# GANtastic3/MaskCycleGAN-VC

Hardware: AMD Instinct MI355X
Metric: train iters/s (full G+D step), 80x64 mel bs=1 (higher is better)
Workload: dtype f32

## Files before the change

include/mcvc.h:

```cpp
#ifndef MCVC_H
#define MCVC_H

#ifdef __cplusplus
extern "C" {
#endif

#define MCVC_ABI_VERSION 3
#define MCVC_GEN_NPARAMS 110
#define MCVC_DISC_NPARAMS 20
#define MCVC_N_MEL 80

int mcvc_version(void);

int mcvc_set_deterministic(int on);
int mcvc_get_deterministic(void);
int mcvc_set_precise(int on);
int mcvc_get_precise(void);
int mcvc_set_trunk_persistent(int on);

int mcvc_twin_begin(void);
int mcvc_twin_switch(void);
int mcvc_twin_end(void);
int mcvc_twin_launches(void);

// ... 125 lines not shown
                     long long scratch_floats, int N, int H, int W, int Cin, int Cout, int branches, int KH, int KW, int stride,
                     int pad_h, int pad_w, int scheme, void* stream);
int mcvc_layer_wgrad(const float* x, const float* dy, float* dw0, float* dw1, float* scratch, long long scratch_floats, int N, int H,
                     int W, int Cin, int Cout, int branches, int KH, int KW, int stride, int pad_h, int pad_w, int scheme, void* stream);
int mcvc_trunk_layer_backward(const float* dy, const float* conv_out, const float* stats, const float* gamma, const float* beta,
                              const float* gamma_gate, const float* beta_gate, const float* w, const float* w_gate, const float* x_in,
                              float* dx, float* dconv, float* dgamma, float* dbeta, float* dgamma_gate, float* dbeta_gate, float* dw,
                              float* dw_gate, float* wpack, int B, int Cin, int T4, int Cout, int KW, void* stream);

int mcvc_instnorm_act_forward(float* x, const float* gamma, const float* beta, const float* gamma_gate,
                              const float* beta_gate, const float* residual, float* y, float* stats,
                              int N, int C, int H, int W, int act, void* stream);
int mcvc_instnorm_act_backward(const float* x, const float* gamma, const float* beta, const float* gamma_gate,
                               const float* beta_gate, const float* stats, float* dy, float* dx,
                               float* dgamma, float* dbeta, float* dgamma_gate, float* dbeta_gate,
                               int N, int C, int H, int W, int act, void* stream);

int mcvc_trunk_layer_forward(const float* x, const float* w, const float* bias, const float* gamma, const float* beta, const float* w_gate,
                             const float* bias_gate, const float* gamma_gate, const float* beta_gate, const float* residual, float* conv_out,
                             float* stats, float* y, int B, int Cin, int T4, int Cout, int KW, void* stream);

int mcvc_batched_gemm(const float* a, const float* b, float* c, int nbatch, int M, int N, int K, int lda, int ldb, int ldc,
                      long long a_stride, long long b_stride, long long c_stride, void* stream);

int mcvc_bias_grad(const float* dy, float* db, int N, int C, int P, void* stream);
int mcvc_act_forward(float* x, float* y, int N, int C, int P, int act, void* stream);
int mcvc_act_backward(const float* x, float* dy, float* dx, int N, int C, int P, int act, void* stream);
int mcvc_fif_input(const float* x, const float* mask, float* xin, int N, int P, void* stream);
int mcvc_fif_input_grad(const float* dxin, const float* mask, float* dx, int N, int P, int accumulate, void* stream);

int mcvc_trace_enable(int on);
int mcvc_trace_kinds(void);
const char* mcvc_trace_kind_name(int kind);
int mcvc_trace_collect(double* out);
int mcvc_trace_collect_raw(double* out, int max_records);

#ifdef __cplusplus
}
#endif
#endif
```

maskcyclegan-vc_amd/csrc/net.hip:

```cpp
#include "mcvc_common.h"
#include "twin.h"
#include "pack.h"
#include "misc.h"
#include "trunk.h"
#include "wino.h"
#include "wino4.h"
#include "sgemm.h"
#include "sampler.h"
#include "audio.h"
#include "../../include/mcvc.h"
#include <string.h>
#include <algorithm>
#include <map>
#include <mutex>
#include <vector>

static int g_deterministic = [] { const char* e = getenv("MCVC_DETERMINISTIC"); return (e && atoi(e) != 0) ? 1 : 0; }();
int mcvc_deterministic() { return g_deterministic; }

namespace {

constexpr float kInEps = 1e-5f;

struct View { float* p; long long sb, sc; int sh; };
// ... 2802 lines not shown
    if (!x || !w || !bias || !gamma || !beta || !conv_out || !stats || !y) return MCVC_ERR_INVALID;
    const int mode = w_gate ? TRUNK_IN_GLU : TRUNK_IN;
    if (!mcvc_trunk_applies(Cin, KW, Cout, B, T4, mode, 1)) return MCVC_ERR_INVALID;
    TrunkArgs a{};
    a.a0 = w; a.bias0 = bias; a.gamma0 = gamma; a.beta0 = beta;
    a.a1 = w_gate; a.bias1 = bias_gate; a.gamma1 = gamma_gate; a.beta1 = beta_gate;
    a.x = x; a.x_sc = (long long)B * T4; a.x_sb = T4;
    a.Cin = Cin; a.KW = KW; a.K = Cin * KW; a.M = Cout; a.Mtot = w_gate ? 2 * Cout : Cout; a.B = B; a.T4 = T4; a.N = B * T4;
    a.conv_out = conv_out; a.c_sc = (long long)B * T4; a.c_sb = T4;
    a.stats = stats; a.y = y; a.res = residual; a.y_sn = T4; a.y_sc = (long long)B * T4; a.eps = kInEps; a.mode = mode;
    return mcvc_trunk_launch(a, 1, (hipStream_t)stream);
}

int mcvc_batched_gemm(const float* a, const float* b, float* c, int nbatch, int M, int N, int K, int lda, int ldb, int ldc,
                      long long a_stride, long long b_stride, long long c_stride, void* stream)
{
    if (!a || !b || !c || nbatch < 1) return MCVC_ERR_INVALID;
    WinoGemmArgs ga{};
    ga.a = a; ga.a_xi = a_stride; ga.lda = lda; ga.b = b; ga.b_xi = b_stride; ga.ldb = ldb; ga.c = c; ga.c_xi = c_stride; ga.ldc = ldc;
    ga.M = M; ga.N = N; ga.K = K; ga.nxi = nbatch;
    return mcvc_wino_gemm_launch(ga, (hipStream_t)stream);
}

int mcvc_bias_grad(const float* dy, float* db, int N, int C, int P, void* stream)
{
    return mcvc_bias_grad_launch(dy, (long long)C * P, (long long)P, N, C, P, db, (hipStream_t)stream);
}

int mcvc_act_forward(float* x, float* y, int N, int C, int P, int act, void* stream)
{
    Exec ex{}; ex.s = (hipStream_t)stream;
    act_fwd(ex, x, 0, 1, y, N, C, P, act);
    return ex.err;
}

int mcvc_act_backward(const float* x, float* dy, float* dx, int N, int C, int P, int act, void* stream)
{
    Exec ex{}; ex.s = (hipStream_t)stream;
    act_bwd(ex, x, dy, 0, 1, dx, N, C, P, act);
    return ex.err;
}

int mcvc_fif_input(const float* x, const float* mask, float* xin, int N, int P, void* stream)
{
    return mcvc_prep_input_launch(x, mask, xin, N, P, (hipStream_t)stream);
}
// ... 8 lines not shown
```

maskcyclegan-vc_amd/csrc/wino.h:

```cpp
#pragma once
#include <hip/hip_runtime.h>

struct WinoXformArgs {
    const float* x; long long x_sb, x_sc; int x_sh;
    float* v;
    int N, C, H, W;
    int TH, TW, NT;
    int NTp;
    int pad;
};

struct WinoOutArgs {
    const float* m;
    const float* bias;
    float* y; long long y_sb, y_sc; int y_sh;
    int N, Cout, OH, OW, TH, TW, NT, NTp;
    int shuffle, YH, YW;
    int accumulate;
};

int mcvc_wino_input_launch(const WinoXformArgs& a, hipStream_t s);
struct NormArgs;
bool mcvc_norm_fwd_wino_applies(const NormArgs& a, const WinoOutArgs& w, int pts);
int mcvc_norm_fwd_wino_launch(const NormArgs& a, const WinoOutArgs& w, int pts, hipStream_t s);
// ... 39 lines not shown
        grow(colv, o);
#pragma unroll
        for (int aa = 0; aa < 6; ++aa) d0[(long long)(aa * 6 + b) * xi_stride] = o[aa];
    }
}
static __device__ __forceinline__ void wino_weight_tile(const float* w, float* dst, int Cout, int Cin, int ld, long long xi_stride, int co_off, int dgrad, int bx, int by)
{
    const int a_idx = bx * 256 + threadIdx.x;
    const int b_idx = by;
    const int co = dgrad ? b_idx : a_idx, ci = dgrad ? a_idx : b_idx;
    if (co >= Cout || ci >= Cin) return;
    wino_weight_core(w + ((long long)co * Cin + ci) * 25, dst, co, ci, ld, xi_stride, co_off, dgrad);
}


struct WinoGemmArgs {
    const float* a; long long a_xi; int lda;
    const float* b; long long b_xi; int ldb;
    float* c; long long c_xi; int ldc;
    int M, N, K;
    int nxi;
    int nt, mt;
    int mgroup;
};
int mcvc_wino_gemm_launch(const WinoGemmArgs& a, hipStream_t s);

template <int P>
static __device__ __forceinline__ void wino_g3(float v0, float v1, float v2, float* o)
{
    if constexpr (P == 4) { o[0] = v0; o[1] = 0.5f * (v0 + v1 + v2); o[2] = 0.5f * (v0 - v1 + v2); o[3] = v2; }
    else {
        const float e = v0 + v2, e2 = v0 * (1.0f / 24.0f) + v2 * (1.0f / 6.0f);
        o[0] = 0.25f * v0; o[1] = -(e + v1) * (1.0f / 6.0f); o[2] = -(e - v1) * (1.0f / 6.0f);
        o[3] = e2 + v1 * (1.0f / 12.0f); o[4] = e2 - v1 * (1.0f / 12.0f); o[5] = v2;
    }
}

template <int P>
static __device__ __forceinline__ void wino3_weight_core_p(const float* g, float* dst, int co, int ci, int ld, long long xi_stride, int co_off)
{
    float gg[5][5];
#pragma unroll
    for (int k = 0; k < 25; ++k) gg[k / 5][k % 5] = g[k];
#pragma unroll
    for (int qh = 0; qh < 2; ++qh)
#pragma unroll
        for (int qw = 0; qw < 2; ++qw) {
            float t[3][P];
// ... 78 lines not shown
```

maskcyclegan-vc_amd/csrc/wino_kernels.hip:

```cpp
#include "mcvc_common.h"
#include "trace.h"
#include "launch.h"
#include "wino.h"

namespace {

__device__ __forceinline__ void bt6(const float d[6], float o[6])
{
    o[0] = 4.f * d[0] - 5.f * d[2] + d[4];
    o[1] = -4.f * (d[1] + d[2]) + d[3] + d[4];
    o[2] = 4.f * (d[1] - d[2]) - d[3] + d[4];
    o[3] = -2.f * d[1] - d[2] + 2.f * d[3] + d[4];
    o[4] = 2.f * d[1] - d[2] - 2.f * d[3] + d[4];
    o[5] = 4.f * d[1] - 5.f * d[3] + d[5];
}

__global__ void __launch_bounds__(256) wino_input_kernel(const Twin<WinoXformArgs> tw)
{
    const WinoXformArgs a = tw.v[blockIdx.z];
    const int tile = blockIdx.x * 256 + threadIdx.x;
    const int c = blockIdx.y;
    if (tile >= a.NT) return;
    const int per = a.TH * a.TW;
    const int n = tile / per, r = tile - n * per;
// ... 434 lines not shown
        float o0, o1;
        at6(u[i], o0, o1);
        const float ov[2] = {o0 + bias, o1 + bias};
        const int oh = 2 * ty + i;
#pragma unroll
        for (int j = 0; j < 2; ++j) {
            const int ow = 2 * tx + j;
            if (oh >= a.OH || ow >= a.OW) continue;
            long long off;
            if (a.shuffle) {
                const int yh = 2 * oh + ((co >> 1) & 1), yw = 2 * ow + (co & 1);
                if (yh >= a.YH || yw >= a.YW) continue;
                off = (long long)(co >> 2) * a.y_sc + (long long)yh * a.y_sh + yw;
            } else {
                off = (long long)co * a.y_sc + (long long)oh * a.y_sh + ow;
            }
            if (a.accumulate) yn[off] += ov[j]; else yn[off] = ov[j];
        }
    }
}


constexpr int kGK = 16;
constexpr int kGStages = 4;
#ifndef MCVC_FOLDK
#define MCVC_FOLDK 32
#endif
constexpr int kFoldK = MCVC_FOLDK;
constexpr int kGA = kGK * 128;

__device__ __forceinline__ void wg_glds16(const float* g, float* l)
{
    __builtin_amdgcn_global_load_lds((const __attribute__((address_space(1))) void*)g,
                                     (__attribute__((address_space(3))) void*)l, 16, 0, 0);
}

template <int BN>
__global__ void __launch_bounds__(256, (BN == 64 ? 3 : 4)) wino_gemm_kernel(const Twin<WinoGemmArgs> tw)
{
    const WinoGemmArgs a = tw.v[blockIdx.z];
    constexpr int kGB = kGK * BN;
    constexpr int kGStage = kGA + kGB;
    constexpr int NACC = (BN == 64) ? 2 : 1;
    extern __shared__ __attribute__((aligned(16))) float smem[];
    const int tid = threadIdx.x, lane = tid & 63;
    const int wave = __builtin_amdgcn_readfirstlane(tid >> 6);
    const int l31 = lane & 31, half = lane >> 5;
    const int wm = (BN == 64) ? (wave >> 1) : wave, wn = (BN == 64) ? (wave & 1) : 0;
    int lid;
    {
        const int total = (int)gridDim.x, linear = (int)blockIdx.x;
        const int q = total >> 3, r = total & 7, xcd = linear & 7, k = linear >> 3;
        lid = (xcd < r ? xcd * (q + 1) : r * (q + 1) + (xcd - r) * q) + k;
    }
    const int n0 = (lid % a.nt) * BN; lid /= a.nt;
    const int m0 = (lid % a.mt) * 128;
    const int xi = lid / a.mt;
    const float* A = a.a + (long long)xi * a.a_xi + m0;
    const float* B = a.b + (long long)xi * a.b_xi + n0;
    const int fa0 = wave * 64 + lane, fa1 = fa0 + 256;
    const float* a_src0 = A + (long long)(fa0 >> 5) * a.lda + 4 * (fa0 & 31);
    const float* a_src1 = A + (long long)(fa1 >> 5) * a.lda + 4 * (fa1 & 31);
    const int bw = (BN == 64) ? wave : (wave & 1);
    const int fb = bw * 64 + lane;
    constexpr int F4R = BN / 4;
    int bcol = 4 * (fb % F4R);
    if (n0 + bcol > a.ldb - 4) bcol = a.ldb - 4 - n0;
    const float* b_src = B + (long long)(fb / F4R) * a.ldb + bcol;
    const long long a_step = (long long)kGK * a.lda, b_step = (long long)kGK * a.ldb;
    auto issue = [&](int stage_k, int buf) {
        float* base = smem + buf * kGStage;
        wg_glds16(a_src0 + stage_k * a_step, base + (wave * 64) * 4);
        wg_glds16(a_src1 + stage_k * a_step, base + (wave * 64 + 256) * 4);
        wg_glds16(b_src + stage_k * b_step, base + kGA + (bw * 64) * 4);
    };
    f32x16 acc[NACC], tot[NACC];
#pragma unroll
    for (int i = 0; i < NACC; ++i)
#pragma unroll
        for (int r = 0; r < 16; ++r) { acc[i][r] = 0.f; tot[i][r] = 0.f; }
    constexpr int kFoldSt = kFoldK / kGK;
    const int nst = a.K / kGK;
#pragma unroll
    for (int s = 0; s < kGStages - 1; ++s)
        if (s < nst) issue(s, s);
    const int a_lane = half * 128 + wm * (32 * NACC) + l31;
    const int b_lane = kGA + half * BN + wn * 32 + l31;
    for (int st = 0; st < nst; ++st) {
        const int newer = (nst - 1 - st) < (kGStages - 2) ? (nst - 1 - st) : (kGStages - 2);
        if (newer >= 2) __builtin_amdgcn_s_waitcnt(0x0F76);
        else if (newer == 1) __builtin_amdgcn_s_waitcnt(0x0F73);
        else __builtin_amdgcn_s_waitcnt(0x0F70);
        __builtin_amdgcn_s_barrier();
        if (st + kGStages - 1 < nst) issue(st + kGStages - 1, (st + kGStages - 1) % kGStages);
        if (st != 0 && (st % kFoldSt) == 0) {
#pragma unroll
            for (int i = 0; i < NACC; ++i)
#pragma unroll
                for (int r = 0; r < 16; ++r) { tot[i][r] += acc[i][r]; acc[i][r] = 0.f; }
        }
        const float* sb = smem + (st % kGStages) * kGStage;
        if constexpr (BN == 64) {
            float a0 = sb[a_lane], a1 = sb[a_lane + 32], b0 = sb[b_lane];
#pragma unroll
            for (int p = 0; p < kGK / 2; ++p) {
                const int q = (p + 1 < kGK / 2) ? p + 1 : p;
                const float na0 = sb[a_lane + q * 256], na1 = sb[a_lane + q * 256 + 32], nb0 = sb[b_lane + q * 2 * BN];
                acc[0] = __builtin_amdgcn_mfma_f32_32x32x2f32(a0, b0, acc[0], 0, 0, 0);
                acc[1] = __builtin_amdgcn_mfma_f32_32x32x2f32(a1, b0, acc[1], 0, 0, 0);
                __builtin_amdgcn_sched_group_barrier(0x100, 3, 0);
                __builtin_amdgcn_sched_group_barrier(0x008, 2, 0);
                a0 = na0; a1 = na1; b0 = nb0;
            }
        } else {
            float a0 = sb[a_lane], b0 = sb[b_lane];
#pragma unroll
            for (int p = 0; p < kGK / 2; ++p) {
                const int q = (p + 1 < kGK / 2) ? p + 1 : p;
                const float na0 = sb[a_lane + q * 256], nb0 = sb[b_lane + q * 2 * BN];
                acc[0] = __builtin_amdgcn_mfma_f32_32x32x2f32(a0, b0, acc[0], 0, 0, 0);
                __builtin_amdgcn_sched_group_barrier(0x100, 2, 0);
                __builtin_amdgcn_sched_group_barrier(0x008, 1, 0);
                a0 = na0; b0 = nb0;
            }
        }
    }
    const int n = n0 + wn * 32 + l31;
    const long long ldc = a.ldc;
    if (n < a.N) {
        float* C = a.c + (long long)xi * a.c_xi + n + (long long)(m0 + wm * (32 * NACC) + 4 * half) * ldc;
#pragma unroll
        for (int i = 0; i < NACC; ++i)
#pragma unroll
            for (int r = 0; r < 16; ++r) C[(long long)(i * 32 + (r & 3) + 8 * (r >> 2)) * ldc] = tot[i][r] + acc[i][r];
    }
}

template <int N> __device__ __forceinline__ void wait_vm() { __builtin_amdgcn_s_waitcnt(0x0F70 | (N & 15) | ((N >> 4) << 14)); }

template <int BM, int BN, int GK, int ST>
__global__ void __launch_bounds__(256) gemm2_kernel(const Twin<WinoGemmArgs> tw)
{
    const WinoGemmArgs a = tw.v[blockIdx.z];
    constexpr int SA = GK * BM, SB = GK * BN, STAGE = SA + SB;
    constexpr bool W22 = (BN % 64) == 0;
    constexpr int NBM = W22 ? BM / 64 : BM / 128, NBN = W22 ? BN / 64 : BN / 32, NACC = NBM * NBN;
    constexpr int NA = (SA / 4 + 255) / 256, NB = (SB / 4 + 255) / 256, ND = NA + NB;
    extern __shared__ __attribute__((aligned(16))) float smem[];
    const int tid = threadIdx.x, lane = tid & 63;
    const int wave = __builtin_amdgcn_readfirstlane(tid >> 6);
    const int l31 = lane & 31, half = lane >> 5;
    const int wm = W22 ? (wave >> 1) : wave, wn = W22 ? (wave & 1) : 0;
    int lid;
    {
        const int total = (int)gridDim.x, linear = (int)blockIdx.x;
        const int q = total >> 3, r = total & 7, xcd = linear & 7, k = linear >> 3;
        lid = (xcd < r ? xcd * (q + 1) : r * (q + 1) + (xcd - r) * q) + k;
    }
    int n_t, m_t, xi;
    if (a.mgroup == 0) { n_t = lid % a.nt; lid /= a.nt; m_t = lid % a.mt; xi = lid / a.mt; }
    else {
        const int mg = a.mgroup, per = a.mt * a.nt;
        int r = lid % per;
        xi = lid / per;
        const int g = r / (mg * a.nt);
        const int gm = (g + 1) * mg <= a.mt ? mg : a.mt - g * mg;
        r -= g * mg * a.nt;
        n_t = r / gm; m_t = g * mg + r % gm;
    }
    const int n0 = n_t * BN, m0 = m_t * BM;
    const float* A = a.a + (long long)xi * a.a_xi + m0;
    const float* B = a.b + (long long)xi * a.b_xi + n0;
    constexpr int A4R = BM / 4, B4R = BN / 4;
    const float* asrc[NA]; int adst[NA];
#pragma unroll
    for (int i = 0; i < NA; ++i) {
        const int f = (tid + i * 256) % (SA / 4);
        asrc[i] = A + (long long)(f / A4R) * a.lda + 4 * (f % A4R);
        adst[i] = (((wave * 64 + i * 256) % (SA / 4))) * 4;
    }
    const float* bsrc[NB]; int bdst[NB];
#pragma unroll
    for (int i = 0; i < NB; ++i) {
        const int f = (tid + i * 256) % (SB / 4);
        int bcol = 4 * (f % B4R);
        if (n0 + bcol > a.ldb - 4) bcol = a.ldb - 4 - n0;
        bsrc[i] = B + (long long)(f / B4R) * a.ldb + bcol;
        bdst[i] = SA + (((wave * 64 + i * 256) % (SB / 4))) * 4;
    }
    const long long a_step = (long long)GK * a.lda, b_step = (long long)GK * a.ldb;
    auto issue = [&](int stage_k, int buf) {
        float* base = smem + buf * STAGE;
#pragma unroll
        for (int i = 0; i < NA; ++i) wg_glds16(asrc[i] + stage_k * a_step, base + adst[i]);
#pragma unroll
        for (int i = 0; i < NB; ++i) wg_glds16(bsrc[i] + stage_k * b_step, base + bdst[i]);
    };
    f32x16 acc[NACC], tot[NACC];
#pragma unroll
    for (int i = 0; i < NACC; ++i)
#pragma unroll
        for (int r = 0; r < 16; ++r) { acc[i][r] = 0.f; tot[i][r] = 0.f; }
    constexpr int kFoldSt = kFoldK / GK;
    const int nst = a.K / GK;
#pragma unroll
    for (int s = 0; s < ST - 1; ++s)
        if (s < nst) issue(s, s);
    const int a_lane = half * BM + wm * (32 * NBM) + l31;
    const int b_lane = SA + half * BN + wn * (32 * NBN) + l31;
    for (int st = 0; st < nst; ++st) {
        const int newer = (nst - 1 - st) < (ST - 2) ? (nst - 1 - st) : (ST - 2);
        if (newer >= 2) wait_vm<2 * ND>(); else if (newer == 1) wait_vm<ND>(); else wait_vm<0>();
        __builtin_amdgcn_s_barrier();
        if (st + ST - 1 < nst) issue(st + ST - 1, (st + ST - 1) % ST);
        if (st != 0 && (st % kFoldSt) == 0) {
#pragma unroll
            for (int i = 0; i < NACC; ++i)
#pragma unroll
                for (int r = 0; r < 16; ++r) { tot[i][r] += acc[i][r]; acc[i][r] = 0.f; }
        }
        const float* sb = smem + (st % ST) * STAGE;
        float av[NBM], bv[NBN];
#pragma unroll
        for (int i = 0; i < NBM; ++i) av[i] = sb[a_lane + 32 * i];
#pragma unroll
        for (int j = 0; j < NBN; ++j) bv[j] = sb[b_lane + 32 * j];
#pragma unroll
        for (int p = 0; p < GK / 2; ++p) {
            const int q = (p + 1 < GK / 2) ? p + 1 : p;
            float na[NBM], nb[NBN];
#pragma unroll
            for (int i = 0; i < NBM; ++i) na[i] = sb[a_lane + q * 2 * BM + 32 * i];
#pragma unroll
            for (int j = 0; j < NBN; ++j) nb[j] = sb[b_lane + q * 2 * BN + 32 * j];
#pragma unroll
            for (int i = 0; i < NBM; ++i)
#pragma unroll
                for (int j = 0; j < NBN; ++j) acc[i * NBN + j] = __builtin_amdgcn_mfma_f32_32x32x2f32(av[i], bv[j], acc[i * NBN + j], 0, 0, 0);
            __builtin_amdgcn_sched_group_barrier(0x100, NBM + NBN, 0);
            __builtin_amdgcn_sched_group_barrier(0x008, NACC, 0);
#pragma unroll
            for (int i = 0; i < NBM; ++i) av[i] = na[i];
#pragma unroll
            for (int j = 0; j < NBN; ++j) bv[j] = nb[j];
        }
    }
    const long long ldc = a.ldc;
    const int Nv = a.N;
    float* Cb = a.c + (long long)xi * a.c_xi + (long long)(m0 + wm * (32 * NBM) + 4 * half) * ldc;
#pragma unroll
    for (int j = 0; j < NBN; ++j) {
        const int n = n0 + wn * (32 * NBN) + 32 * j + l31;
        if (n >= Nv) continue;
        float* C = Cb + n;
#pragma unroll
        for (int i = 0; i < NBM; ++i)
#pragma unroll
            for (int r = 0; r < 16; ++r) C[(long long)(i * 32 + (r & 3) + 8 * (r >> 2)) * ldc] = tot[i * NBN + j][r] + acc[i * NBN + j][r];
    }
}

template <int BM, int BN, int GK, int ST>
static int gemm2_launch(WinoGemmArgs b, int nxi, hipStream_t s)
{
    if ((b.M % BM) != 0 || (b.K % GK) != 0) return MCVC_ERR_INVALID;
    b.nt = cdiv_i(b.N, BN); b.mt = b.M / BM;
    {
        static const int mgk = mcvc_knob("MCVC_GEMM_MGROUP", 8);
        static const int mgn = mcvc_knob("MCVC_GEMM_MGROUP_MINNT", 8);
        b.mgroup = (mgk > 0 && b.nt >= mgn) ? (mgk < b.mt ? mgk : b.mt) : 0;
    }
    constexpr size_t lds = (size_t)ST * (GK * BM + GK * BN) * sizeof(float);
    static bool done = false;
    if (!done) {
        hipError_t e = hipFuncSetAttribute(reinterpret_cast<const void*>(gemm2_kernel<BM, BN, GK, ST>), hipFuncAttributeMaxDynamicSharedMemorySize, 160 * 1024);
        if (e != hipSuccess) return (int)e;
        done = true;
    }
    mcvc_launch((gemm2_kernel<BM, BN, GK, ST>), dim3((unsigned)(b.nt * b.mt * nxi)), dim3(256), lds, s, b);
    return (int)hipGetLastError();
}

}

int mcvc_wino_input_launch(const WinoXformArgs& a, hipStream_t s)
{
    dim3 grid((unsigned)cdiv_i(a.NT, 256), (unsigned)a.C);
    TraceScope ts(K_ELEMENTWISE, s, 0.0, 4.0 * ((double)a.N * a.C * a.H * a.W + 36.0 * a.C * a.NT));
    mcvc_launch(wino_input_kernel, grid, dim3(256), 0, s, a);
    return (int)hipGetLastError();
}

int mcvc_wino_output_launch(const WinoOutArgs& a, hipStream_t s)
{
    dim3 grid((unsigned)cdiv_i(a.NT, 256), (unsigned)a.Cout);
    TraceScope ts(K_ELEMENTWISE, s, 0.0, 4.0 * (36.0 * a.Cout * a.NT + 4.0 * a.Cout * a.NT));
    mcvc_launch(wino_output_kernel, grid, dim3(256), 0, s, a);
    return (int)hipGetLastError();
}

int mcvc_wino_gemm_launch(const WinoGemmArgs& a, hipStream_t s)
{
    if ((a.K % kGK) != 0 || (a.M % 128) != 0 || (a.lda & 3) || (a.ldb & 3) || a.ldb < 64) return MCVC_ERR_INVALID;
    const int nxi = a.nxi > 0 ? a.nxi : 36;
    WinoGemmArgs b = a;
    static const int knob = mcvc_knob("MCVC_WINO_BN", 0);
    const int pad64 = cdiv_i(a.N, 64) * 64, pad32 = cdiv_i(a.N, 32) * 32;
    bool narrow = (pad64 * 10 > pad32 * 11) && a.N <= 512 && a.ldb >= 32;
    if (knob == 32) narrow = a.ldb >= 32; else if (knob == 64) narrow = false;
    b.mt = a.M / 128;
    TraceScope ts(K_WINO_GEMM, s, 2.0 * nxi * a.M * a.N * a.K, 4.0 * nxi * ((double)a.K * a.M + (double)a.K * a.N + (double)a.M * a.N));
#ifdef MCVC_EXPERIMENTS
    static const int cfg2 = mcvc_knob("MCVC_GEMM_CFG", 0);
    static const bool verbose = mcvc_knob_set("MCVC_GEMM_VERBOSE");
    if (verbose && mcvc_twin_phase() != 1) fprintf(stderr, "[gemm] nxi=%d M=%d N=%d K=%d lda=%d ldb=%d twin=%d\n", nxi, a.M, a.N, a.K, a.lda, a.ldb, mcvc_twin_phase() == 2);
    switch (cfg2) {
        case 1: return gemm2_launch<128, 64, 16, 4>(b, nxi, s);
        case 2: return gemm2_launch<128, 32, 16, 4>(b, nxi, s);
        case 3: return gemm2_launch<64, 64, 16, 4>(b, nxi, s);
        case 4: return gemm2_launch<128, 64, 32, 3>(b, nxi, s);
        case 5: return gemm2_launch<128, 32, 32, 3>(b, nxi, s);
        case 6: return gemm2_launch<64, 64, 32, 3>(b, nxi, s);
        case 7: return gemm2_launch<128, 64, 16, 6>(b, nxi, s);
        case 8: return gemm2_launch<128, 32, 16, 6>(b, nxi, s);
        case 9: return gemm2_launch<64, 64, 16, 6>(b, nxi, s);
        case 10: return gemm2_launch<128, 64, 32, 4>(b, nxi, s);
        case 11: return gemm2_launch<64, 64, 32, 4>(b, nxi, s);
        case 12: return gemm2_launch<128, 128, 16, 4>(b, nxi, s);
        case 13: return gemm2_launch<128, 128, 32, 3>(b, nxi, s);
        case 14: return gemm2_launch<128, 128, 16, 6>(b, nxi, s);
        case 15: return gemm2_launch<128, 128, 32, 2>(b, nxi, s);
        default: break;
    }
#else
    constexpr int cfg2 = 0;
#endif
    static const int big = mcvc_knob("MCVC_GEMM_BIG", 1);
    if (cfg2 == 0 && big && a.N >= 1280 && (a.K % 16) == 0 && (long long)cdiv_i(a.N, 128) * (a.M / 128) * nxi >= 1280)
        return gemm2_launch<128, 128, 16, 4>(b, nxi, s);
    auto rounds_cost = [&](int bm, int bn) { return (double)cdiv_i(cdiv_i(a.N, bn) * (a.M / bm) * nxi, 256) * bm * bn; };
    static const int costsel = mcvc_knob("MCVC_GEMM_COST", 1);
    if (cfg2 == 0 && a.K >= 512 && (a.K % 32) == 0 && (a.M % 64) == 0) {
        if (!(costsel && a.ldb >= 32 && rounds_cost(128, 32) < 0.94 * rounds_cost(64, 64))) return gemm2_launch<64, 64, 32, 4>(b, nxi, s);
        return gemm2_launch<128, 32, 16, 4>(b, nxi, s);
    }
    if (narrow) {
        b.nt = cdiv_i(a.N, 32);
        static bool done = false;
        if (!done) {
            hipError_t e = hipFuncSetAttribute(reinterpret_cast<const void*>(wino_gemm_kernel<32>), hipFuncAttributeMaxDynamicSharedMemorySize, 64 * 1024);
            if (e != hipSuccess) return (int)e;
            done = true;
        }
        mcvc_launch(wino_gemm_kernel<32>, dim3((unsigned)(b.nt * b.mt * nxi)), dim3(256), (size_t)kGStages * (kGA + kGK * 32) * sizeof(float), s, b);
    } else {
        b.nt = cdiv_i(a.N, 64);
        mcvc_launch(wino_gemm_kernel<64>, dim3((unsigned)(b.nt * b.mt * nxi)), dim3(256), (size_t)kGStages * (kGA + kGK * 64) * sizeof(float), s, b);
    }
    return (int)hipGetLastError();
}

int mcvc_wino_input_t_launch(const WinoXformArgs& a, hipStream_t s)
{
    return xform_t_launch<0>(a, 0, 0, 4.0 * ((double)a.N * a.C * a.H * a.W + 36.0 * a.C * a.NTp), s);
}

int mcvc_wino_dy_t_launch(const WinoXformArgs& a, hipStream_t s)
{
    return xform_t_launch<1>(a, 0, 0, 4.0 * ((double)a.N * a.C * a.H * a.W + 36.0 * a.C * a.NTp), s);
}

int mcvc_wino_dw_launch(const float* du, float* dw, int Cout, int Cin, hipStream_t s)
{
    dim3 grid((unsigned)cdiv_i(Cin, 256), (unsigned)Cout);
    TraceScope ts(K_ELEMENTWISE, s, 0.0, 4.0 * (36.0 + 50.0) * Cout * Cin);
    mcvc_launch(wino_dw_kernel, grid, dim3(256), 0, s, WinoDwKArgs{du, dw, Cout, Cin});
    return (int)hipGetLastError();
}

int mcvc_wino3_input_launch(const WinoXformArgs& a, hipStream_t s)
{
    dim3 grid((unsigned)cdiv_i(a.NT, 256), (unsigned)a.C);
// ... 39 lines not shown
```

maskcyclegan-vc_amd/mask_cyclegan_vc/_hip.py:

```python
from __future__ import annotations

import ctypes
import os
from ctypes import c_float, c_int, c_longlong, c_void_p

import torch

_HERE = os.path.dirname(os.path.abspath(__file__))
LIB_PATH = os.environ.get("MCVC_LIB") or os.path.join(os.path.dirname(_HERE), "lib", "libmcvc_hip.so")

ABI_VERSION = 3
GEN_NPARAMS = 110
DISC_NPARAMS = 20
N_MEL = 80

_lib = None

_PP = ctypes.POINTER(c_void_p)

_SIGS = {
    "mcvc_version": (c_int, []),
    "mcvc_set_deterministic": (c_int, [c_int]),
    "mcvc_get_deterministic": (c_int, []),
    "mcvc_set_precise": (c_int, [c_int]),
# ... 63 lines not shown
                                ctypes.c_ulonglong, ctypes.c_ulonglong, c_void_p, c_void_p, c_void_p, c_void_p, c_void_p, c_void_p]),
    "mcvc_audio_frames": (c_int, [c_int]),
    "mcvc_audio_basis_floats": (c_longlong, []),
    "mcvc_audio_basis_init": (c_int, [c_void_p]),
    "mcvc_audio_plan": (c_int, [c_void_p, c_int, c_void_p, c_void_p, c_int, ctypes.POINTER(c_int)]),
    "mcvc_audio_log_mel": (c_int, [c_void_p, c_longlong, c_void_p, c_int, c_void_p, c_void_p, c_longlong, c_void_p]),
    "mcvc_axpy": (c_int, [c_void_p, c_void_p, c_float, c_longlong, c_void_p]),
    "mcvc_conv2d_pack_floats": (c_longlong, [c_int, c_int, c_int, c_int]),
    "mcvc_conv2d_forward": (c_int, [c_void_p] * 6 + [c_int] * 12 + [c_void_p]),
    "mcvc_conv2d_dgrad": (c_int, [c_void_p] * 5 + [c_int] * 11 + [c_void_p]),
    "mcvc_conv2d_wgrad_slab_floats": (c_longlong, [c_int] * 10),
    "mcvc_conv2d_wgrad": (c_int, [c_void_p] * 4 + [c_longlong] + [c_int] * 10 + [c_void_p]),
    "mcvc_layer_packed_floats": (c_longlong, [c_int] * 8),
    "mcvc_layer_scratch_floats": (c_longlong, [c_int] * 11),
    "mcvc_layer_pack": (c_int, [c_void_p] * 5 + [c_int] * 8 + [c_void_p]),
    "mcvc_layer_forward": (c_int, [c_void_p] * 6 + [c_longlong] + [c_int] * 13 + [c_void_p]),
    "mcvc_layer_dgrad": (c_int, [c_void_p] * 6 + [c_longlong] + [c_int] * 12 + [c_void_p]),
    "mcvc_layer_wgrad": (c_int, [c_void_p] * 5 + [c_longlong] + [c_int] * 12 + [c_void_p]),
    "mcvc_trunk_layer_backward": (c_int, [c_void_p] * 19 + [c_int] * 5 + [c_void_p]),
    "mcvc_instnorm_act_forward": (c_int, [c_void_p] * 8 + [c_int] * 5 + [c_void_p]),
    "mcvc_instnorm_act_backward": (c_int, [c_void_p] * 12 + [c_int] * 5 + [c_void_p]),
    "mcvc_trunk_layer_forward": (c_int, [c_void_p] * 13 + [c_int] * 5 + [c_void_p]),
    "mcvc_batched_gemm": (c_int, [c_void_p] * 3 + [c_int] * 7 + [c_longlong] * 3 + [c_void_p]),
    "mcvc_bias_grad": (c_int, [c_void_p, c_void_p, c_int, c_int, c_int, c_void_p]),
    "mcvc_act_forward": (c_int, [c_void_p, c_void_p, c_int, c_int, c_int, c_int, c_void_p]),
    "mcvc_act_backward": (c_int, [c_void_p, c_void_p, c_void_p, c_int, c_int, c_int, c_int, c_void_p]),
    "mcvc_fif_input": (c_int, [c_void_p, c_void_p, c_void_p, c_int, c_int, c_void_p]),
    "mcvc_fif_input_grad": (c_int, [c_void_p, c_void_p, c_void_p, c_int, c_int, c_int, c_void_p]),
    "mcvc_trace_enable": (c_int, [c_int]),
    "mcvc_trace_kinds": (c_int, []),
    "mcvc_trace_kind_name": (ctypes.c_char_p, [c_int]),
    "mcvc_trace_collect": (c_int, [ctypes.POINTER(ctypes.c_double)]),
    "mcvc_trace_collect_raw": (c_int, [ctypes.POINTER(ctypes.c_double), c_int]),
}

EXPORTED_SYMBOLS = tuple(_SIGS)


def lib():
    global _lib
    if _lib is None:
        if not os.path.exists(LIB_PATH):
            raise RuntimeError(
                "libmcvc_hip.so not found at %s -- build it with `python -c 'import __graft_entry__ as g; g.build()'` "
                "(hipcc --offload-arch=gfx950). There is no CPU fallback." % LIB_PATH)
        L = ctypes.CDLL(LIB_PATH)
# ... 56 lines not shown
```

Before: 177.2.

## Make Winograd GEMM persistent with occupancy-sized grid and cost-based tile choice

Converts the gemm2 kernel into a persistent kernel: a grid sized from occupancy (halved under twin streams, optionally capped) loops over output tiles either contiguously or strided, pipelining loads of the next tile across tile boundaries and overlapping the previous tile's stores with waitcnt accounting. The older wino_gemm_kernel path is removed, and tile shape selection now uses a cost model based on rounds per slot and the CU count. It also exports knobs for setting the workgroup cap and querying the chosen plan. The aim is to cut tail effects and launch-wave quantization on small GEMMs. In exchange it adds per-tile address recomputation, more complex vmcnt waits, and possible load imbalance.

```diff
diff --git a/include/mcvc.h b/include/mcvc.h
--- a/include/mcvc.h
+++ b/include/mcvc.h
@@ -171,6 +171,8 @@
 
 int mcvc_batched_gemm(const float* a, const float* b, float* c, int nbatch, int M, int N, int K, int lda, int ldb, int ldc,
                       long long a_stride, long long b_stride, long long c_stride, void* stream);
+int mcvc_set_gemm_workgroups(int n);
+int mcvc_gemm_plan(int nbatch, int M, int N, int K, int ldb);
 
 int mcvc_bias_grad(const float* dy, float* db, int N, int C, int P, void* stream);
 int mcvc_act_forward(float* x, float* y, int N, int C, int P, int act, void* stream);
diff --git a/maskcyclegan-vc_amd/csrc/net.hip b/maskcyclegan-vc_amd/csrc/net.hip
--- a/maskcyclegan-vc_amd/csrc/net.hip
+++ b/maskcyclegan-vc_amd/csrc/net.hip
@@ -2848,6 +2848,9 @@
     return mcvc_wino_gemm_launch(ga, (hipStream_t)stream);
 }
 
+int mcvc_set_gemm_workgroups(int n) { return mcvc_wino_gemm_set_workgroups(n); }
+int mcvc_gemm_plan(int nbatch, int M, int N, int K, int ldb) { return mcvc_wino_gemm_plan(nbatch, M, N, K, ldb); }
+
 int mcvc_bias_grad(const float* dy, float* db, int N, int C, int P, void* stream)
 {
     return mcvc_bias_grad_launch(dy, (long long)C * P, (long long)P, N, C, P, db, (hipStream_t)stream);
diff --git a/maskcyclegan-vc_amd/csrc/wino.h b/maskcyclegan-vc_amd/csrc/wino.h
--- a/maskcyclegan-vc_amd/csrc/wino.h
+++ b/maskcyclegan-vc_amd/csrc/wino.h
@@ -85,8 +85,12 @@
     int nxi;
     int nt, mt;
     int mgroup;
+    int ntiles;
+    int contig;
 };
 int mcvc_wino_gemm_launch(const WinoGemmArgs& a, hipStream_t s);
+int mcvc_wino_gemm_set_workgroups(int n);
+int mcvc_wino_gemm_plan(int nxi, int M, int N, int K, int ldb);
 
 template <int P>
 static __device__ __forceinline__ void wino_g3(float v0, float v1, float v2, float* o)
diff --git a/maskcyclegan-vc_amd/csrc/wino_kernels.hip b/maskcyclegan-vc_amd/csrc/wino_kernels.hip
--- a/maskcyclegan-vc_amd/csrc/wino_kernels.hip
+++ b/maskcyclegan-vc_amd/csrc/wino_kernels.hip
@@ -480,118 +480,15 @@
 
 
 constexpr int kGK = 16;
-constexpr int kGStages = 4;
 #ifndef MCVC_FOLDK
 #define MCVC_FOLDK 32
 #endif
 constexpr int kFoldK = MCVC_FOLDK;
-constexpr int kGA = kGK * 128;
 
 __device__ __forceinline__ void wg_glds16(const float* g, float* l)
 {
     __builtin_amdgcn_global_load_lds((const __attribute__((address_space(1))) void*)g,
                                      (__attribute__((address_space(3))) void*)l, 16, 0, 0);
-}
-
-template <int BN>
-__global__ void __launch_bounds__(256, (BN == 64 ? 3 : 4)) wino_gemm_kernel(const Twin<WinoGemmArgs> tw)
-{
-    const WinoGemmArgs a = tw.v[blockIdx.z];
-    constexpr int kGB = kGK * BN;
-    constexpr int kGStage = kGA + kGB;
-    constexpr int NACC = (BN == 64) ? 2 : 1;
-    extern __shared__ __attribute__((aligned(16))) float smem[];
-    const int tid = threadIdx.x, lane = tid & 63;
-    const int wave = __builtin_amdgcn_readfirstlane(tid >> 6);
-    const int l31 = lane & 31, half = lane >> 5;
-    const int wm = (BN == 64) ? (wave >> 1) : wave, wn = (BN == 64) ? (wave & 1) : 0;
-    int lid;
-    {
-        const int total = (int)gridDim.x, linear = (int)blockIdx.x;
-        const int q = total >> 3, r = total & 7, xcd = linear & 7, k = linear >> 3;
-        lid = (xcd < r ? xcd * (q + 1) : r * (q + 1) + (xcd - r) * q) + k;
-    }
-    const int n0 = (lid % a.nt) * BN; lid /= a.nt;
-    const int m0 = (lid % a.mt) * 128;
-    const int xi = lid / a.mt;
-    const float* A = a.a + (long long)xi * a.a_xi + m0;
-    const float* B = a.b + (long long)xi * a.b_xi + n0;
-    const int fa0 = wave * 64 + lane, fa1 = fa0 + 256;
-    const float* a_src0 = A + (long long)(fa0 >> 5) * a.lda + 4 * (fa0 & 31);
-    const float* a_src1 = A + (long long)(fa1 >> 5) * a.lda + 4 * (fa1 & 31);
-    const int bw = (BN == 64) ? wave : (wave & 1);
-    const int fb = bw * 64 + lane;
-    constexpr int F4R = BN / 4;
-    int bcol = 4 * (fb % F4R);
-    if (n0 + bcol > a.ldb - 4) bcol = a.ldb - 4 - n0;
-    const float* b_src = B + (long long)(fb / F4R) * a.ldb + bcol;
-    const long long a_step = (long long)kGK * a.lda, b_step = (long long)kGK * a.ldb;
-    auto issue = [&](int stage_k, int buf) {
-        float* base = smem + buf * kGStage;
-        wg_glds16(a_src0 + stage_k * a_step, base + (wave * 64) * 4);
-        wg_glds16(a_src1 + stage_k * a_step, base + (wave * 64 + 256) * 4);
-        wg_glds16(b_src + stage_k * b_step, base + kGA + (bw * 64) * 4);
-    };
-    f32x16 acc[NACC], tot[NACC];
-#pragma unroll
-    for (int i = 0; i < NACC; ++i)
-#pragma unroll
-        for (int r = 0; r < 16; ++r) { acc[i][r] = 0.f; tot[i][r] = 0.f; }
-    constexpr int kFoldSt = kFoldK / kGK;
-    const int nst = a.K / kGK;
-#pragma unroll
-    for (int s = 0; s < kGStages - 1; ++s)
-        if (s < nst) issue(s, s);
-    const int a_lane = half * 128 + wm * (32 * NACC) + l31;
-    const int b_lane = kGA + half * BN + wn * 32 + l31;
-    for (int st = 0; st < nst; ++st) {
-        const int newer = (nst - 1 - st) < (kGStages - 2) ? (nst - 1 - st) : (kGStages - 2);
-        if (newer >= 2) __builtin_amdgcn_s_waitcnt(0x0F76);
-        else if (newer == 1) __builtin_amdgcn_s_waitcnt(0x0F73);
-        else __builtin_amdgcn_s_waitcnt(0x0F70);
-        __builtin_amdgcn_s_barrier();
-        if (st + kGStages - 1 < nst) issue(st + kGStages - 1, (st + kGStages - 1) % kGStages);
-        if (st != 0 && (st % kFoldSt) == 0) {
-#pragma unroll
-            for (int i = 0; i < NACC; ++i)
-#pragma unroll
-                for (int r = 0; r < 16; ++r) { tot[i][r] += acc[i][r]; acc[i][r] = 0.f; }
-        }
-        const float* sb = smem + (st % kGStages) * kGStage;
-        if constexpr (BN == 64) {
-            float a0 = sb[a_lane], a1 = sb[a_lane + 32], b0 = sb[b_lane];
-#pragma unroll
-            for (int p = 0; p < kGK / 2; ++p) {
-                const int q = (p + 1 < kGK / 2) ? p + 1 : p;
-                const float na0 = sb[a_lane + q * 256], na1 = sb[a_lane + q * 256 + 32], nb0 = sb[b_lane + q * 2 * BN];
-                acc[0] = __builtin_amdgcn_mfma_f32_32x32x2f32(a0, b0, acc[0], 0, 0, 0);
-                acc[1] = __builtin_amdgcn_mfma_f32_32x32x2f32(a1, b0, acc[1], 0, 0, 0);
-                __builtin_amdgcn_sched_group_barrier(0x100, 3, 0);
-                __builtin_amdgcn_sched_group_barrier(0x008, 2, 0);
-                a0 = na0; a1 = na1; b0 = nb0;
-            }
-        } else {
-            float a0 = sb[a_lane], b0 = sb[b_lane];
-#pragma unroll
-            for (int p = 0; p < kGK / 2; ++p) {
-                const int q = (p + 1 < kGK / 2) ? p + 1 : p;
-                const float na0 = sb[a_lane + q * 256], nb0 = sb[b_lane + q * 2 * BN];
-                acc[0] = __builtin_amdgcn_mfma_f32_32x32x2f32(a0, b0, acc[0], 0, 0, 0);
-                __builtin_amdgcn_sched_group_barrier(0x100, 2, 0);
-                __builtin_amdgcn_sched_group_barrier(0x008, 1, 0);
-                a0 = na0; b0 = nb0;
-            }
-        }
-    }
-    const int n = n0 + wn * 32 + l31;
-    const long long ldc = a.ldc;
-    if (n < a.N) {
-        float* C = a.c + (long long)xi * a.c_xi + n + (long long)(m0 + wm * (32 * NACC) + 4 * half) * ldc;
-#pragma unroll
-        for (int i = 0; i < NACC; ++i)
-#pragma unroll
-            for (int r = 0; r < 16; ++r) C[(long long)(i * 32 + (r & 3) + 8 * (r >> 2)) * ldc] = tot[i][r] + acc[i][r];
-    }
 }
 
 template <int N> __device__ __forceinline__ void wait_vm() { __builtin_amdgcn_s_waitcnt(0x0F70 | (N & 15) | ((N >> 4) << 14)); }
@@ -604,80 +501,134 @@
     constexpr bool W22 = (BN % 64) == 0;
     constexpr int NBM = W22 ? BM / 64 : BM / 128, NBN = W22 ? BN / 64 : BN / 32, NACC = NBM * NBN;
     constexpr int NA = (SA / 4 + 255) / 256, NB = (SB / 4 + 255) / 256, ND = NA + NB;
+    constexpr int NS = 16 * NACC;
+    constexpr int VMAX = 63;
     extern __shared__ __attribute__((aligned(16))) float smem[];
     const int tid = threadIdx.x, lane = tid & 63;
     const int wave = __builtin_amdgcn_readfirstlane(tid >> 6);
     const int l31 = lane & 31, half = lane >> 5;
     const int wm = W22 ? (wave >> 1) : wave, wn = W22 ? (wave & 1) : 0;
-    int lid;
+    int t0, tstep, cnt;
     {
         const int total = (int)gridDim.x, linear = (int)blockIdx.x;
         const int q = total >> 3, r = total & 7, xcd = linear & 7, k = linear >> 3;
-        lid = (xcd < r ? xcd * (q + 1) : r * (q + 1) + (xcd - r) * q) + k;
-    }
-    int n_t, m_t, xi;
-    if (a.mgroup == 0) { n_t = lid % a.nt; lid /= a.nt; m_t = lid % a.mt; xi = lid / a.mt; }
-    else {
-        const int mg = a.mgroup, per = a.mt * a.nt;
-        int r = lid % per;
-        xi = lid / per;
-        const int g = r / (mg * a.nt);
-        const int gm = (g + 1) * mg <= a.mt ? mg : a.mt - g * mg;
-        r -= g * mg * a.nt;
-        n_t = r / gm; m_t = g * mg + r % gm;
-    }
-    const int n0 = n_t * BN, m0 = m_t * BM;
-    const float* A = a.a + (long long)xi * a.a_xi + m0;
-    const float* B = a.b + (long long)xi * a.b_xi + n0;
+        const int w = (xcd < r ? xcd * (q + 1) : r * (q + 1) + (xcd - r) * q) + k;
+        if (a.contig) {
+            const int tq = a.ntiles / total, tr = a.ntiles - tq * total;
+            t0 = w * tq + (w < tr ? w : tr); tstep = 1; cnt = tq + (w < tr ? 1 : 0);
+        } else { t0 = w; tstep = total; cnt = (a.ntiles - w + total - 1) / total; }
+    }
+    if (cnt <= 0) return;
+    auto decode = [&](int lid, int& n0, int& m0, int& xi) {
+        int n_t, m_t;
+        if (a.mgroup == 0) { n_t = lid % a.nt; lid /= a.nt; m_t = lid % a.mt; xi = lid / a.mt; }
+        else {
+            const int mg = a.mgroup, per = a.mt * a.nt;
+            int r = lid % per;
+            xi = lid / per;
+            const int g = r / (mg * a.nt);
+            const int gm = (g + 1) * mg <= a.mt ? mg : a.mt - g * mg;
+            r -= g * mg * a.nt;
+            n_t = r / gm; m_t = g * mg + r % gm;
+        }
+        n0 = n_t * BN; m0 = m_t * BM;
+    };
     constexpr int A4R = BM / 4, B4R = BN / 4;
     const float* asrc[NA]; int adst[NA];
-#pragma unroll
-    for (int i = 0; i < NA; ++i) {
-        const int f = (tid + i * 256) % (SA / 4);
-        asrc[i] = A + (long long)(f / A4R) * a.lda + 4 * (f % A4R);
-        adst[i] = (((wave * 64 + i * 256) % (SA / 4))) * 4;
-    }
     const float* bsrc[NB]; int bdst[NB];
 #pragma unroll
-    for (int i = 0; i < NB; ++i) {
-        const int f = (tid + i * 256) % (SB / 4);
-        int bcol = 4 * (f % B4R);
-        if (n0 + bcol > a.ldb - 4) bcol = a.ldb - 4 - n0;
-        bsrc[i] = B + (long long)(f / B4R) * a.ldb + bcol;
-        bdst[i] = SA + (((wave * 64 + i * 256) % (SB / 4))) * 4;
-    }
-    const long long a_step = (long long)GK * a.lda, b_step = (long long)GK * a.ldb;
-    auto issue = [&](int stage_k, int buf) {
-        float* base = smem + buf * STAGE;
-#pragma unroll
-        for (int i = 0; i < NA; ++i) wg_glds16(asrc[i] + stage_k * a_step, base + adst[i]);
-#pragma unroll
-        for (int i = 0; i < NB; ++i) wg_glds16(bsrc[i] + stage_k * b_step, base + bdst[i]);
+    for (int i = 0; i < NA; ++i) adst[i] = (((wave * 64 + i * 256) % (SA / 4))) * 4;
+#pragma unroll
+    for (int i = 0; i < NB; ++i) bdst[i] = SA + (((wave * 64 + i * 256) % (SB / 4))) * 4;
+    const int lda = a.lda, ldb = a.ldb;
+    auto set_tile = [&](int t) {
+        int n0, m0, xi;
+        decode(t, n0, m0, xi);
+        const float* A = a.a + (long long)xi * a.a_xi + m0;
+        const float* B = a.b + (long long)xi * a.b_xi + n0;
+#pragma unroll
+        for (int i = 0; i < NA; ++i) {
+            const int f = (tid + i * 256) % (SA / 4);
+            asrc[i] = A + (long long)(f / A4R) * lda + 4 * (f % A4R);
+        }
+#pragma unroll
+        for (int i = 0; i < NB; ++i) {
+            const int f = (tid + i * 256) % (SB / 4);
+            int bcol = 4 * (f % B4R);
+            if (n0 + bcol > ldb - 4) bcol = ldb - 4 - n0;
+            bsrc[i] = B + (long long)(f / B4R) * ldb + bcol;
+        }
+    };
+    const long long a_step = (long long)GK * lda, b_step = (long long)GK * ldb;
+    const int nst = a.K / GK;
+    const int total = cnt * nst;
+    int it = 0, ik = 0, ib = 0;
+    set_tile(t0);
+    auto issue_next = [&]() {
+        float* base = smem + ib * STAGE;
+#pragma unroll
+        for (int i = 0; i < NA; ++i) wg_glds16(asrc[i] + ik * a_step, base + adst[i]);
+#pragma unroll
+        for (int i = 0; i < NB; ++i) wg_glds16(bsrc[i] + ik * b_step, base + bdst[i]);
+        ib = (ib + 1 == ST) ? 0 : ib + 1;
+        if (++ik == nst) {
+            ik = 0;
+            if (++it < cnt) set_tile(t0 + it * tstep);
+        }
     };
     f32x16 acc[NACC], tot[NACC];
 #pragma unroll
     for (int i = 0; i < NACC; ++i)
 #pragma unroll
         for (int r = 0; r < 16; ++r) { acc[i][r] = 0.f; tot[i][r] = 0.f; }
+    const long long ldc = a.ldc;
+    const int Nv = a.N;
+    auto store_tile = [&](int t) -> bool {
+        int n0, m0, xi;
+        decode(t, n0, m0, xi);
+        float* Cb = a.c + (long long)xi * a.c_xi + (long long)(m0 + wm * (32 * NBM) + 4 * half) * ldc;
+        const int nw = n0 + wn * (32 * NBN);
+        const bool full = nw + 32 * NBN <= Nv;
+#pragma unroll
+        for (int j = 0; j < NBN; ++j) {
+            const int n = nw + 32 * j + l31;
+            float* C = Cb + n;
+#pragma unroll
+            for (int i = 0; i < NBM; ++i)
+#pragma unroll
+                for (int r = 0; r < 16; ++r) {
+                    const float v = tot[i * NBN + j][r] + acc[i * NBN + j][r];
+                    if (full || n < Nv) C[(long long)(i * 32 + (r & 3) + 8 * (r >> 2)) * ldc] = v;
+                    acc[i * NBN + j][r] = 0.f; tot[i * NBN + j][r] = 0.f;
+                }
+        }
+        return full;
+    };
     constexpr int kFoldSt = kFoldK / GK;
-    const int nst = a.K / GK;
 #pragma unroll
     for (int s = 0; s < ST - 1; ++s)
-        if (s < nst) issue(s, s);
+        if (s < total) issue_next();
     const int a_lane = half * BM + wm * (32 * NBM) + l31;
     const int b_lane = SA + half * BN + wn * (32 * NBN) + l31;
-    for (int st = 0; st < nst; ++st) {
-        const int newer = (nst - 1 - st) < (ST - 2) ? (nst - 1 - st) : (ST - 2);
-        if (newer >= 2) wait_vm<2 * ND>(); else if (newer == 1) wait_vm<ND>(); else wait_vm<0>();
+    int ct = 0, ks = 0, cb = 0;
+    int since = ST;
+    for (int g = 0; g < total; ++g) {
+        const int newer = (total - 1 - g) < (ST - 2) ? (total - 1 - g) : (ST - 2);
+        const bool st_newer = since < ST;
+        if (newer >= 2) { if (st_newer) wait_vm<(2 * ND + NS > VMAX ? VMAX : 2 * ND + NS)>(); else wait_vm<2 * ND>(); }
+        else if (newer == 1) { if (st_newer) wait_vm<(ND + NS > VMAX ? VMAX : ND + NS)>(); else wait_vm<ND>(); }
+        else { if (st_newer) wait_vm<(NS > VMAX ? VMAX : NS)>(); else wait_vm<0>(); }
         __builtin_amdgcn_s_barrier();
-        if (st + ST - 1 < nst) issue(st + ST - 1, (st + ST - 1) % ST);
-        if (st != 0 && (st % kFoldSt) == 0) {
+        if (g + ST - 1 < total) issue_next();
+        ++since;
+        if (ks == 0 && g != 0) since = store_tile(t0 + (ct - 1) * tstep) ? 1 : ST;
+        else if (ks != 0 && (ks % kFoldSt) == 0) {
 #pragma unroll
             for (int i = 0; i < NACC; ++i)
 #pragma unroll
                 for (int r = 0; r < 16; ++r) { tot[i][r] += acc[i][r]; acc[i][r] = 0.f; }
         }
-        const float* sb = smem + (st % ST) * STAGE;
+        const float* sb = smem + cb * STAGE;
         float av[NBM], bv[NBN];
 #pragma unroll
         for (int i = 0; i < NBM; ++i) av[i] = sb[a_lane + 32 * i];
@@ -702,40 +653,55 @@
 #pragma unroll
             for (int j = 0; j < NBN; ++j) bv[j] = nb[j];
         }
-    }
-    const long long ldc = a.ldc;
-    const int Nv = a.N;
-    float* Cb = a.c + (long long)xi * a.c_xi + (long long)(m0 + wm * (32 * NBM) + 4 * half) * ldc;
-#pragma unroll
-    for (int j = 0; j < NBN; ++j) {
-        const int n = n0 + wn * (32 * NBN) + 32 * j + l31;
-        if (n >= Nv) continue;
-        float* C = Cb + n;
-#pragma unroll
-        for (int i = 0; i < NBM; ++i)
-#pragma unroll
-            for (int r = 0; r < 16; ++r) C[(long long)(i * 32 + (r & 3) + 8 * (r >> 2)) * ldc] = tot[i * NBN + j][r] + acc[i * NBN + j][r];
-    }
+        cb = (cb + 1 == ST) ? 0 : cb + 1;
+        if (++ks == nst) { ks = 0; ++ct; }
+    }
+    store_tile(t0 + (ct - 1) * tstep);
+}
+
+int g_gemm_wg_cap = 0;
+
+template <int BM, int BN, int GK, int ST>
+static int gemm2_slots()
+{
+    static int slots = 0;
+    if (slots == 0) {
+        constexpr size_t lds = (size_t)ST * (GK * BM + GK * BN) * sizeof(float);
+        const void* fn = reinterpret_cast<const void*>(gemm2_kernel<BM, BN, GK, ST>);
+        int dev = 0, ncu = 0, per = 0;
+        if (hipFuncSetAttribute(fn, hipFuncAttributeMaxDynamicSharedMemorySize, 160 * 1024) != hipSuccess || hipGetDevice(&dev) != hipSuccess ||
+            hipDeviceGetAttribute(&ncu, hipDeviceAttributeMultiprocessorCount, dev) != hipSuccess ||
+            hipOccupancyMaxActiveBlocksPerMultiprocessor(&per, fn, 256, lds) != hipSuccess || ncu < 1 || per < 1) return -1;
+        slots = ncu * per;
+    }
+    return slots;
+}
+
+static int gemm2_grid(int ntiles, int slots)
+{
+    int g = slots / (mcvc_twin_phase() != 0 ? 2 : 1);
+    if (g_gemm_wg_cap > 0 && g > g_gemm_wg_cap) g = g_gemm_wg_cap;
+    if (g > ntiles) g = ntiles;
+    return g < 1 ? 1 : g;
 }
 
 template <int BM, int BN, int GK, int ST>
 static int gemm2_launch(WinoGemmArgs b, int nxi, hipStream_t s)
 {
-    if ((b.M % BM) != 0 || (b.K % GK) != 0) return MCVC_ERR_INVALID;
+    if ((b.M % BM) != 0 || (b.K % GK) != 0 || b.K < GK) return MCVC_ERR_INVALID;
     b.nt = cdiv_i(b.N, BN); b.mt = b.M / BM;
+    b.ntiles = b.nt * b.mt * nxi;
     {
         static const int mgk = mcvc_knob("MCVC_GEMM_MGROUP", 8);
         static const int mgn = mcvc_knob("MCVC_GEMM_MGROUP_MINNT", 8);
         b.mgroup = (mgk > 0 && b.nt >= mgn) ? (mgk < b.mt ? mgk : b.mt) : 0;
+        static const int contig = mcvc_knob("MCVC_GEMM_CONTIG", 0);
+        b.contig = contig;
     }
     constexpr size_t lds = (size_t)ST * (GK * BM + GK * BN) * sizeof(float);
-    static bool done = false;
-    if (!done) {
-        hipError_t e = hipFuncSetAttribute(reinterpret_cast<const void*>(gemm2_kernel<BM, BN, GK, ST>), hipFuncAttributeMaxDynamicSharedMemorySize, 160 * 1024);
-        if (e != hipSuccess) return (int)e;
-        done = true;
-    }
-    mcvc_launch((gemm2_kernel<BM, BN, GK, ST>), dim3((unsigned)(b.nt * b.mt * nxi)), dim3(256), lds, s, b);
+    const int slots = gemm2_slots<BM, BN, GK, ST>();
+    if (slots <= 0) return MCVC_ERR_INVALID;
+    mcvc_launch((gemm2_kernel<BM, BN, GK, ST>), dim3((unsigned)gemm2_grid(b.ntiles, slots)), dim3(256), lds, s, b);
     return (int)hipGetLastError();
 }
 
@@ -757,65 +723,96 @@
     return (int)hipGetLastError();
 }
 
+namespace {
+struct GemmTile { int bm, bn, gk, st; };
+constexpr GemmTile kT64x64{64, 64, 32, 4}, kT128x32{128, 32, 16, 4}, kT128x64{128, 64, 16, 4}, kT128x128{128, 128, 16, 4};
+
+static int gemm_tile_slots(const GemmTile& t)
+{
+    if (t.bm == 64) return gemm2_slots<64, 64, 32, 4>();
+    if (t.bn == 32) return gemm2_slots<128, 32, 16, 4>();
+    if (t.bn == 64) return gemm2_slots<128, 64, 16, 4>();
+    return gemm2_slots<128, 128, 16, 4>();
+}
+
+static double gemm_tile_cost(const GemmTile& t, int nxi, int M, int N, int K)
+{
+    const int slots = gemm_tile_slots(t);
+    if (slots <= 0) return 1e300;
+    static int ncu = 0;
+    if (ncu == 0) { int dev = 0; if (hipGetDevice(&dev) != hipSuccess || hipDeviceGetAttribute(&ncu, hipDeviceAttributeMultiprocessorCount, dev) != hipSuccess) ncu = 256; }
+    const int ntiles = cdiv_i(N, t.bn) * (M / t.bm) * nxi, g = gemm2_grid(ntiles, slots);
+    const int nets = mcvc_twin_phase() != 0 ? 2 : 1;
+    return (double)cdiv_i(ntiles, g) * K * t.bm * t.bn * cdiv_i(g * nets, ncu);
+}
+
+static GemmTile gemm_choose(int nxi, int M, int N, int K, int ldb)
+{
+    static const int big = mcvc_knob("MCVC_GEMM_BIG", 1);
+    if (big && N >= 1280 && (long long)cdiv_i(N, 128) * (M / 128) * nxi >= 1280) return kT128x128;
+    static const int costsel = mcvc_knob("MCVC_GEMM_COST", 1);
+    const bool longk = K >= 512 && (K % 32) == 0;
+    GemmTile best = longk ? kT64x64 : kT128x64;
+    double cbest = gemm_tile_cost(best, nxi, M, N, K) * (longk ? 0.94 : 1.0);
+    if (!costsel && longk) return best;
+    for (const GemmTile& t : {kT128x32, kT128x64}) {
+        if (t.bn == best.bn && t.bm == best.bm) continue;
+        if (t.bn == 32 && ldb < 32) continue;
+        const double c = gemm_tile_cost(t, nxi, M, N, K);
+        if (c < cbest) { best = t; cbest = c; }
+    }
+    return best;
+}
+
+static int gemm_tile_launch(const GemmTile& t, const WinoGemmArgs& b, int nxi, hipStream_t s)
+{
+    if (t.bm == 64) return gemm2_launch<64, 64, 32, 4>(b, nxi, s);
+    if (t.bn == 32) return gemm2_launch<128, 32, 16, 4>(b, nxi, s);
+    if (t.bn == 64) return gemm2_launch<128, 64, 16, 4>(b, nxi, s);
+    return gemm2_launch<128, 128, 16, 4>(b, nxi, s);
+}
+}
+
+int mcvc_wino_gemm_set_workgroups(int n) { const int was = g_gemm_wg_cap; g_gemm_wg_cap = n > 0 ? n : 0; return was; }
+
+int mcvc_wino_gemm_plan(int nxi, int M, int N, int K, int ldb)
+{
+    if (nxi < 1 || M < 128 || (M % 128) != 0 || N < 1 || K < kGK || (K % kGK) != 0 || ldb < 64) return -1;
+    const GemmTile t = gemm_choose(nxi, M, N, K, ldb);
+    return (t.bm << 16) | (t.bn << 8) | t.gk;
+}
+
 int mcvc_wino_gemm_launch(const WinoGemmArgs& a, hipStream_t s)
 {
-    if ((a.K % kGK) != 0 || (a.M % 128) != 0 || (a.lda & 3) || (a.ldb & 3) || a.ldb < 64) return MCVC_ERR_INVALID;
+    if ((a.K % kGK) != 0 || a.K < kGK || (a.M % 128) != 0 || (a.lda & 3) || (a.ldb & 3) || a.ldb < 64) return MCVC_ERR_INVALID;
     const int nxi = a.nxi > 0 ? a.nxi : 36;
-    WinoGemmArgs b = a;
-    static const int knob = mcvc_knob("MCVC_WINO_BN", 0);
-    const int pad64 = cdiv_i(a.N, 64) * 64, pad32 = cdiv_i(a.N, 32) * 32;
-    bool narrow = (pad64 * 10 > pad32 * 11) && a.N <= 512 && a.ldb >= 32;
-    if (knob == 32) narrow = a.ldb >= 32; else if (knob == 64) narrow = false;
-    b.mt = a.M / 128;
     TraceScope ts(K_WINO_GEMM, s, 2.0 * nxi * a.M * a.N * a.K, 4.0 * nxi * ((double)a.K * a.M + (double)a.K * a.N + (double)a.M * a.N));
 #ifdef MCVC_EXPERIMENTS
     static const int cfg2 = mcvc_knob("MCVC_GEMM_CFG", 0);
     static const bool verbose = mcvc_knob_set("MCVC_GEMM_VERBOSE");
+    static const int wgcap = mcvc_knob("MCVC_GEMM_WG", -1);
+    if (wgcap >= 0) g_gemm_wg_cap = wgcap;
     if (verbose && mcvc_twin_phase() != 1) fprintf(stderr, "[gemm] nxi=%d M=%d N=%d K=%d lda=%d ldb=%d twin=%d\n", nxi, a.M, a.N, a.K, a.lda, a.ldb, mcvc_twin_phase() == 2);
     switch (cfg2) {
-        case 1: return gemm2_launch<128, 64, 16, 4>(b, nxi, s);
-        case 2: return gemm2_launch<128, 32, 16, 4>(b, nxi, s);
-        case 3: return gemm2_launch<64, 64, 16, 4>(b, nxi, s);
-        case 4: return gemm2_launch<128, 64, 32, 3>(b, nxi, s);
-        case 5: return gemm2_launch<128, 32, 32, 3>(b, nxi, s);
-        case 6: return gemm2_launch<64, 64, 32, 3>(b, nxi, s);
-        case 7: return gemm2_launch<128, 64, 16, 6>(b, nxi, s);
-        case 8: return gemm2_launch<128, 32, 16, 6>(b, nxi, s);
-        case 9: return gemm2_launch<64, 64, 16, 6>(b, nxi, s);
-        case 10: return gemm2_launch<128, 64, 32, 4>(b, nxi, s);
-        case 11: return gemm2_launch<64, 64, 32, 4>(b, nxi, s);
-        case 12: return gemm2_launch<128, 128, 16, 4>(b, nxi, s);
-        case 13: return gemm2_launch<128, 128, 32, 3>(b, nxi, s);
-        case 14: return gemm2_launch<128, 128, 16, 6>(b, nxi, s);
-        case 15: return gemm2_launch<128, 128, 32, 2>(b, nxi, s);
+        case 1: return gemm2_launch<128, 64, 16, 4>(a, nxi, s);
+        case 2: return gemm2_launch<128, 32, 16, 4>(a, nxi, s);
+        case 3: return gemm2_launch<64, 64, 16, 4>(a, nxi, s);
+        case 4: return gemm2_launch<128, 64, 32, 3>(a, nxi, s);
+        case 5: return gemm2_launch<128, 32, 32, 3>(a, nxi, s);
+        case 6: return gemm2_launch<64, 64, 32, 3>(a, nxi, s);
+        case 7: return gemm2_launch<128, 64, 16, 6>(a, nxi, s);
+        case 8: return gemm2_launch<128, 32, 16, 6>(a, nxi, s);
+        case 9: return gemm2_launch<64, 64, 16, 6>(a, nxi, s);
+        case 10: return gemm2_launch<128, 64, 32, 4>(a, nxi, s);
+        case 11: return gemm2_launch<64, 64, 32, 4>(a, nxi, s);
+        case 12: return gemm2_launch<128, 128, 16, 4>(a, nxi, s);
+        case 13: return gemm2_launch<128, 128, 32, 3>(a, nxi, s);
+        case 14: return gemm2_launch<128, 128, 16, 6>(a, nxi, s);
+        case 15: return gemm2_launch<128, 128, 32, 2>(a, nxi, s);
         default: break;
     }
-#else
-    constexpr int cfg2 = 0;
 #endif
-    static const int big = mcvc_knob("MCVC_GEMM_BIG", 1);
-    if (cfg2 == 0 && big && a.N >= 1280 && (a.K % 16) == 0 && (long long)cdiv_i(a.N, 128) * (a.M / 128) * nxi >= 1280)
-        return gemm2_launch<128, 128, 16, 4>(b, nxi, s);
-    auto rounds_cost = [&](int bm, int bn) { return (double)cdiv_i(cdiv_i(a.N, bn) * (a.M / bm) * nxi, 256) * bm * bn; };
-    static const int costsel = mcvc_knob("MCVC_GEMM_COST", 1);
-    if (cfg2 == 0 && a.K >= 512 && (a.K % 32) == 0 && (a.M % 64) == 0) {
-        if (!(costsel && a.ldb >= 32 && rounds_cost(128, 32) < 0.94 * rounds_cost(64, 64))) return gemm2_launch<64, 64, 32, 4>(b, nxi, s);
-        return gemm2_launch<128, 32, 16, 4>(b, nxi, s);
-    }
-    if (narrow) {
-        b.nt = cdiv_i(a.N, 32);
-        static bool done = false;
-        if (!done) {
-            hipError_t e = hipFuncSetAttribute(reinterpret_cast<const void*>(wino_gemm_kernel<32>), hipFuncAttributeMaxDynamicSharedMemorySize, 64 * 1024);
-            if (e != hipSuccess) return (int)e;
-            done = true;
-        }
-        mcvc_launch(wino_gemm_kernel<32>, dim3((unsigned)(b.nt * b.mt * nxi)), dim3(256), (size_t)kGStages * (kGA + kGK * 32) * sizeof(float), s, b);
-    } else {
-        b.nt = cdiv_i(a.N, 64);
-        mcvc_launch(wino_gemm_kernel<64>, dim3((unsigned)(b.nt * b.mt * nxi)), dim3(256), (size_t)kGStages * (kGA + kGK * 64) * sizeof(float), s, b);
-    }
-    return (int)hipGetLastError();
+    return gemm_tile_launch(gemm_choose(nxi, a.M, a.N, a.K, a.ldb), a, nxi, s);
 }
 
 int mcvc_wino_input_t_launch(const WinoXformArgs& a, hipStream_t s)
diff --git a/maskcyclegan-vc_amd/mask_cyclegan_vc/_hip.py b/maskcyclegan-vc_amd/mask_cyclegan_vc/_hip.py
--- a/maskcyclegan-vc_amd/mask_cyclegan_vc/_hip.py
+++ b/maskcyclegan-vc_amd/mask_cyclegan_vc/_hip.py
@@ -109,6 +109,8 @@
     "mcvc_instnorm_act_backward": (c_int, [c_void_p] * 12 + [c_int] * 5 + [c_void_p]),
     "mcvc_trunk_layer_forward": (c_int, [c_void_p] * 13 + [c_int] * 5 + [c_void_p]),
     "mcvc_batched_gemm": (c_int, [c_void_p] * 3 + [c_int] * 7 + [c_longlong] * 3 + [c_void_p]),
+    "mcvc_set_gemm_workgroups": (c_int, [c_int]),
+    "mcvc_gemm_plan": (c_int, [c_int] * 5),
     "mcvc_bias_grad": (c_int, [c_void_p, c_void_p, c_int, c_int, c_int, c_void_p]),
     "mcvc_act_forward": (c_int, [c_void_p, c_void_p, c_int, c_int, c_int, c_int, c_void_p]),
     "mcvc_act_backward": (c_int, [c_void_p, c_void_p, c_void_p, c_int, c_int, c_int, c_int, c_void_p]),
```

New measurement: 167.7. -5.4%, worse.
